# sizhe-li/neural-jacobian-field

Hardware: AMD Instinct MI355X
Metric: rendered rays/s (64 samples/ray, 256^2 image) (higher is better)
Workload: dtype f32 (v_mfma_f32_32x32x2_f32: exact fp32 products, fp32 accumulate -- the reference's arithmetic)

## Files before the change

### neural-jacobian-field_amd/csrc/njf_device.h

```cpp
#pragma once
#include <hip/hip_runtime.h>
#include <stdint.h>

__device__ __forceinline__ float relu_bits(float x) { return __int_as_float(max(__float_as_int(x), 0)); }

typedef float f32x16 __attribute__((ext_vector_type(16)));
typedef float f32x4 __attribute__((ext_vector_type(4)));
typedef _Float16 f16x8 __attribute__((ext_vector_type(8)));
typedef _Float16 f16x16 __attribute__((ext_vector_type(16)));
typedef _Float16 f16x32 __attribute__((ext_vector_type(32)));
typedef int i32x8 __attribute__((ext_vector_type(8)));
typedef int i32x4 __attribute__((ext_vector_type(4)));
typedef int i32x2 __attribute__((ext_vector_type(2)));
typedef unsigned u32x6 __attribute__((ext_vector_type(6)));

#define PREC_F32 0
#define PREC_F16X2 1
#define PREC_F16F6 2
#define PREC_F16 3

#define NJF_WAVES 4
#define NJF_THREADS (NJF_WAVES * 64)
#define NJF_CHUNK 8192

// ... 674 lines not shown
#pragma unroll
      for (int e = 0; e < 4; ++e) {
        if (t == 0) {
          h[m][4 * q + e] = fmaf(v[b % DEPTH][q][e], w[0], h[m][4 * q + e]);
        } else {
          float acc = h[m][4 * q + e];
          asm("v_fmac_f32 %0, %1, %2" : "+v"(acc) : "v"(v[b % DEPTH][q][e]), "v"(w[t]));
          h[m][4 * q + e] = acc;
        }
      }
    asm volatile("" : "+v"(h[m]) : : "memory");
    if (b + DEPTH < NB) issue(b + DEPTH);
    __builtin_amdgcn_sched_barrier(0);
  }
}

#define NJF_F16_GATHER_DEPTH 8
template <int MB, int DEPTH = NJF_F16_GATHER_DEPTH>
__device__ __forceinline__ void add_hoisted_latent_f16(const _Float16* __restrict__ gz, const PointGeom& g, int hh,
                                                       f32x16 (&h)[MB], const Footprint* shared = nullptr) {
  if (!NJF_GATHER) return;
  Footprint f;
  if (shared != nullptr) f = *shared;
  else point_footprint(g, f);
  const _Float16* gb = gz + (size_t)g.gofs + 8 * hh;
  const _Float16* p[4] = {gb + f.t00, gb + f.t01, gb + f.t10, gb + f.t11};
  const float w[4] = {f.w00, f.w01, f.w10, f.w11};
  constexpr int NB = 4 * MB;
  constexpr int D = DEPTH < NB ? DEPTH : NB;
  f16x8 v[D][2];
  auto issue = [&](int b) {
    const _Float16* src = p[b / MB] + 32 * (b % MB);
#pragma unroll
    for (int q = 0; q < 2; ++q) v[b % D][q] = *(const f16x8*)(src + 16 * q);
  };
#pragma unroll
  for (int b = 0; b < D; ++b) issue(b);
#pragma unroll
  for (int b = 0; b < NB; ++b) {
    const int t = b / MB, m = b % MB;
#pragma unroll
    for (int q = 0; q < 2; ++q)
#pragma unroll
      for (int e = 0; e < 8; ++e) h[m][8 * q + e] = fmaf((float)v[b % D][q][e], w[t], h[m][8 * q + e]);
    asm volatile("" : "+v"(h[m]) : : "memory");
    if (b + D < NB) issue(b + D);
    __builtin_amdgcn_sched_barrier(0);
  }
}

struct TileShareF16 {
  unsigned pe[16];
};

__device__ __forceinline__ void share_tile(const f32x16 (&pe)[2], TileShareF16& sh) {
#pragma unroll
  for (int t = 0; t < 4; ++t)
#pragma unroll
    for (int p = 0; p < 4; ++p) sh.pe[4 * t + p] = pack_pair_f16<false>(pe[t >> 1][8 * (t & 1) + 2 * p], pe[t >> 1][8 * (t & 1) + 2 * p + 1]);
}

template <class ST>
__device__ __forceinline__ void mma_lin_in_f16_packed(ST& st, const float* __restrict__ wl, int lane, const unsigned (&pk)[16],
                                                      f32x16 (&out)[4]) {
  const f16x8* base = (const f16x8*)wl + lane;
  constexpr int T = 4;
  f16x8 a[4];
#pragma unroll
  for (int i = 0; i < 4; ++i) a[i] = base[i * 64];
#pragma unroll
  for (int t = 0; t < T; ++t) {
    f16x8 n[4] = {a[0], a[1], a[2], a[3]};
    if (t + 1 < T) {
#pragma unroll
      for (int i = 0; i < 4; ++i) n[i] = base[((t + 1) * 4 + i) * 64];
    }
    dma_issue(st, 2 * t);
    dma_issue(st, 2 * t + 1);
    __builtin_amdgcn_sched_barrier(0);
    const f16x8 b = __builtin_bit_cast(f16x8, u32x4{pk[4 * t], pk[4 * t + 1], pk[4 * t + 2], pk[4 * t + 3]});
#pragma unroll
    for (int m = 0; m < 4; ++m) out[m] = __builtin_amdgcn_mfma_f32_32x32x16_f16(a[m], b, out[m], 0, 0, 0);
#pragma unroll
    for (int i = 0; i < 4; ++i) a[i] = n[i];
  }
}


template <int MB, int PREC, int DEPTH = 4>
__device__ __forceinline__ void add_hoisted_latent(const float* __restrict__ gz, const PointGeom& g, int lane,
                                                   f32x16 (&h)[MB]) {
  if constexpr (PREC == PREC_F16) add_hoisted_latent_f16<MB>((const _Float16*)gz, g, lane >> 5, h);
  else if constexpr (PREC == PREC_F16F6) add_hoisted_latent_quad<MB, DEPTH>(gz, g, lane, h);
  else add_hoisted_latent_half<MB, DEPTH>(gz, g, lane >> 5, h);
}

template <int PREC>
__device__ __forceinline__ const float* map_at(const float* base, size_t elements) {
  if constexpr (PREC == PREC_F16) return (const float*)((const _Float16*)base + elements);
  else return base + elements;
}

__device__ __forceinline__ float sin_accurate(float arg) {
  const float C_HI = 0.15915493667125702f, C_LO = 6.4206382432985265e-09f;
  const float u = arg * C_HI;
  float e = fmaf(arg, C_HI, -u);
  e = fmaf(arg, C_LO, e);
  const float y = (u - rintf(u)) + e;
  return __builtin_amdgcn_sinf(y);
}

__device__ __forceinline__ void positional_encoding(float xc, float yc, float zc, int hh, f32x16 (&pe)[2]) {
#ifdef NJF_ABLATE_PE
  pe[0] = (f32x16)(xc);
  pe[1] = (f32x16)(yc + zc);
  return;
#endif
  const float two_pi = 6.2831855f;
  const float half_pi = hh ? 1.5707964f : 0.0f;
  const float sx[3] = {two_pi * xc, two_pi * yc, two_pi * zc};
#pragma unroll
  for (int s = 0; s < 30; ++s) {
    const int d = s / 10, f = s % 10;
    const float arg = sx[d] * (float)(1 << f) + half_pi;
    pe[s >> 4][s & 15] = sin_accurate(arg);
  }
  pe[1][14] = hh ? zc : xc;
  pe[1][15] = hh ? 1.0f : yc;
}

__device__ __forceinline__ void sh4(float dx, float dy, float dz, float (&o)[16]) {
  const float x = ((dx + 1.0f) / 2.0f) * 2.0f - 1.0f;
  const float y = ((dy + 1.0f) / 2.0f) * 2.0f - 1.0f;
  const float z = ((dz + 1.0f) / 2.0f) * 2.0f - 1.0f;
  const float xy = x * y, xz = x * z, yz = y * z, x2 = x * x, y2 = y * y, z2 = z * z;
  o[0] = 0.28209479177387814f;
  o[1] = -0.48860251190291987f * y;
  o[2] = 0.48860251190291987f * z;
  o[3] = -0.48860251190291987f * x;
  o[4] = 1.0925484305920792f * xy;
  o[5] = -1.0925484305920792f * yz;
  o[6] = 0.94617469575755997f * z2 - 0.31539156525251999f;
  o[7] = -1.0925484305920792f * xz;
  o[8] = 0.54627421529603959f * x2 - 0.54627421529603959f * y2;
  o[9] = 0.59004358992664352f * y * (-3.0f * x2 + y2);
  o[10] = 2.8906114426405538f * xy * z;
  o[11] = 0.45704579946446572f * y * (1.0f - 5.0f * z2);
  o[12] = 0.3731763325901154f * z * (5.0f * z2 - 3.0f);
  o[13] = 0.45704579946446572f * x * (1.0f - 5.0f * z2);
  o[14] = 1.4453057213202769f * z * (x2 - y2);
  o[15] = 0.59004358992664352f * x * (-x2 + 3.0f * y2);
}

template <int KB0, bool RELU, int KBI, class ST>
__device__ __forceinline__ void mma_chunk_gather_f32(ST& st, const float* __restrict__ wl, int lane, const f32x16 (&in)[KBI],
                                                     f32x16 (&out)[4], const float* __restrict__ gz, const PointGeom& g) {
  static_assert(NJF_DMA_ROUNDS == 8, "one DMA round behind every second group of blocks 0 and 1");
  constexpr int DEPTH = 2;
  constexpr int FIRST = 4;
  Footprint f;
  point_footprint(g, f);
  const float* gb = gz + (size_t)g.gofs + 4 * (lane >> 5);
  const float* p[4] = {gb + f.t00, gb + f.t01, gb + f.t10, gb + f.t11};
  const float w[4] = {f.w00, f.w01, f.w10, f.w11};
  f32x4 v[DEPTH][4];
  auto issue = [&](int b) {
    const float* src = p[b & 3] + 32 * (b >> 2);
#pragma unroll
    for (int q = 0; q < 4; ++q) v[b % DEPTH][q] = *(const f32x4*)(src + 8 * q);
  };
  auto fold = [&](int m, int i) {
    const int t = i >> 4, r = i & 15, b = 4 * m + t;
    if (t == 0) {
      out[m][r] = fmaf(v[b % DEPTH][r >> 2][r & 3], w[0], out[m][r]);
    } else {
      float acc = out[m][r];
      asm("v_fmac_f32 %0, %1, %2" : "+v"(acc) : "v"(v[b % DEPTH][r >> 2][r & 3]), "v"(w[t]));
      out[m][r] = acc;
    }
  };
  auto refill = [&](int m, int t) {
    asm volatile("" : "+v"(out[m]) : : "memory");
    if (4 * m + t + DEPTH < 16) issue(4 * m + t + DEPTH);
  };
  auto folded = [](int n) { return n <= FIRST ? 0 : (n - FIRST) * 64 / (32 - FIRST); };
  if (NJF_GATHER) {
#pragma unroll
    for (int b = 0; b < DEPTH; ++b) issue(b);
  }
  const float* base = wl + lane * 4;
  f32x16 bin[2];
  f32x4 a = *(const f32x4*)base;
#pragma unroll
  for (int m = 0; m < 4; ++m) {
#pragma unroll
    for (int kq = 0; kq < 8; ++kq) {
      const int kb = kq >> 2, q = kq & 3, gi = 8 * m + kq;
      f32x4 n = a;
      if (gi + 1 < 32) n = *(const f32x4*)(base + (((gi + 1) & 7) * 4 + ((gi + 1) >> 3)) * 256);
      if (gi < 16 && (gi & 1) == 0) dma_issue(st, gi >> 1);
#pragma unroll
      for (int e = 0; e < 4; ++e) {
        if (m == 0) {
          float b = in[KB0 + kb][q * 4 + e];
          if (RELU) b = relu_bits(b);
          bin[kb][q * 4 + e] = b;
        }
        out[m] = __builtin_amdgcn_mfma_f32_32x32x2f32(a[e], bin[kb][q * 4 + e], out[m], 0, 0, 0);
        if (NJF_GATHER && m > 0) {
#pragma unroll
          for (int i = folded(4 * kq + e); i < folded(4 * kq + e + 1); ++i) fold(m - 1, i);
        }
      }
      if (NJF_GATHER && m > 0) {
#pragma unroll
        for (int t = folded(4 * kq) / 16; t < folded(4 * kq + 4) / 16; ++t) refill(m - 1, t);
      }
      a = n;
      __builtin_amdgcn_sched_barrier(0);
    }
  }
  st.dma_next = NJF_DMA_ROUNDS;
  NJF_STAMP(st, 4);
  if (NJF_GATHER) {
#pragma unroll
    for (int t = 0; t < 4; ++t) {
#pragma unroll
      for (int i = 16 * t; i < 16 * t + 16; ++i) fold(3, i);
      refill(3, t);
      __builtin_amdgcn_sched_barrier(0);
    }
  }
  NJF_STAMP(st, 5);
}

struct ActDump {
  float* act;
  float* pe;
  size_t stride;
  unsigned* mask = nullptr;
  bool half = false;
  float* feat = nullptr;
};

__device__ __forceinline__ float* dump_layer(const ActDump& d, int l) {
  if (d.act == nullptr) return nullptr;
  return d.half ? (float*)((_Float16*)d.act + (size_t)l * d.stride) : d.act + (size_t)l * d.stride;
}

template <bool DO_RELU>
__device__ __forceinline__ void dump_vec128(float* __restrict__ dst, const f32x16 (&v)[4], unsigned* __restrict__ mask = nullptr,
                                            bool half = false) {
  if (dst == nullptr) return;
  if (half) {
    _Float16* d16 = (_Float16*)dst;
#pragma unroll
    for (int m = 0; m < 4; ++m)
#pragma unroll
      for (int q = 0; q < 2; ++q) {
        u32x4 o;
#pragma unroll
        for (int e = 0; e < 4; ++e) o[e] = pack_pair_f16<DO_RELU>(v[m][8 * q + 2 * e], v[m][8 * q + 2 * e + 1]);
        *(u32x4*)(d16 + 16 * m + 8 * q) = o;
      }
  } else {
#pragma unroll
  for (int m = 0; m < 4; ++m)
#pragma unroll
    for (int q = 0; q < 4; ++q) {
      f32x4 o;
#pragma unroll
      for (int e = 0; e < 4; ++e) o[e] = DO_RELU ? fmaxf(v[m][4 * q + e], 0.f) : v[m][4 * q + e];
      *(f32x4*)(dst + 16 * m + 4 * q) = o;
    }
  }
  if (mask != nullptr) {
    unsigned w[2] = {0u, 0u};
#pragma unroll
    for (int m = 0; m < 4; ++m)
#pragma unroll
      for (int r = 0; r < 16; ++r) {
        const unsigned b = (unsigned)min(max(__float_as_int(v[m][r]), 0), 1);
        w[m >> 1] |= b << (16 * (m & 1) + r);
      }
    typedef unsigned u32x2 __attribute__((ext_vector_type(2)));
    *(u32x2*)mask = u32x2{w[0], w[1]};
  }
}

template <int PREC, bool DUMP = false, int SHARED = 0, class ST>
__device__ __forceinline__ void resnet_tile(ST& st, const float* __restrict__ bias,
                                            const float* __restrict__ gz, const PointGeom& g,
                                            const f32x16 (&pe)[2], int wave, int lane, f32x16 (&out)[1],
                                            ActDump dump = ActDump{nullptr, nullptr, 0}, const TileShareF16* share = nullptr) {
  static_assert(SHARED == 0 || (PREC == PREC_F16 && !DUMP), "the shared tile state exists for the plain-fp16 inference kernels");
  const int hh = lane >> 5;
  constexpr bool FUSED = PREC == PREC_F32 && !DUMP;
  f32x16 h[4], net[4];
#pragma unroll
  for (int m = 0; m < 4; ++m) h[m] = (f32x16)(0.f);
  if (DUMP && dump.pe != nullptr) {
#pragma unroll
    for (int kb = 0; kb < 2; ++kb)
#pragma unroll
      for (int q = 0; q < 4; ++q) {
        f32x4 o;
#pragma unroll
        for (int e = 0; e < 4; ++e) o[e] = pe[kb][4 * q + e];
        *(f32x4*)(dump.pe + 16 * kb + 4 * q) = o;
      }
  }
  {
    const float* wl = stream_step(st, wave, lane);
    if constexpr ((SHARED & 1) != 0) mma_lin_in_f16_packed(st, wl, lane, share->pe, h);
    else if constexpr (FUSED) mma_chunk_gather_f32<0, false, 2>(st, wl, lane, pe, h, gz, g);
    else mma_chunk<PREC, 4, 2, 0, false, 2>(st, wl, lane, pe, h);
  }
  if constexpr (PREC == PREC_F16) {
    static_assert(!DUMP, "the plain-fp16 mode is an inference mode (training forwards dump fp32-class activations)");
    Footprint fp_net;
    if constexpr ((SHARED & 2) != 0) point_footprint(g, fp_net);
    for (int blk = 0; blk < 5; ++blk) {
      if (blk < 3) {
        NJF_STAMP(st, 4);
        if constexpr ((SHARED & 2) != 0) add_hoisted_latent_f16<4>((const _Float16*)map_at<PREC>(gz, blk * 128), g, hh, h, &fp_net);
        else add_hoisted_latent<4, PREC>(map_at<PREC>(gz, blk * 128), g, lane, h);
        NJF_STAMP(st, 5);
      }
      const float* bl = bias + blk * 256;
      bias_init<4, true, PREC>(bl, hh, net);
      {
        const float* wl = stream_step(st, wave, lane);
        mma_chunk<PREC, 4, 4, 0, true, 4>(st, wl, lane, h, net);
      }
      if (blk >= 2) bias_init<4, false, PREC, true>(bl + 128, hh, h);
      {
        const float* wl = stream_step(st, wave, lane);
        mma_chunk<PREC, 4, 4, 0, true, 4>(st, wl, lane, net, h);
      }
    }
  } else
  for (int blk = 0; blk < 5; ++blk) {
    if (!FUSED && blk < 3) {
      NJF_STAMP(st, 4);
      add_hoisted_latent<4, PREC>(gz + blk * 128, g, lane, h);
      NJF_STAMP(st, 5);
    }
    if (DUMP) dump_vec128<true>(dump_layer(dump, 2 * blk), h, dump.mask ? dump.mask + (size_t)(2 * blk) * (dump.stride / 32) : nullptr, dump.half);
    const float* bl = bias + blk * 256;
    bias_init<4, true, PREC>(bl, hh, net);
    {
      {
        const float* wl = stream_step(st, wave, lane);
        mma_chunk<PREC, 4, 2, 0, true, 4>(st, wl, lane, h, net);
      }
      {
        const float* wl = stream_step(st, wave, lane);
        mma_chunk<PREC, 4, 2, 2, true, 4>(st, wl, lane, h, net);
      }
    }
    if (DUMP) dump_vec128<true>(dump_layer(dump, 2 * blk + 1), net, dump.mask ? dump.mask + (size_t)(2 * blk + 1) * (dump.stride / 32) : nullptr, dump.half);
    bias_init<4, false, PREC>(bl + 128, hh, h);
    {
      {
        const float* wl = stream_step(st, wave, lane);
        mma_chunk<PREC, 4, 2, 0, true, 4>(st, wl, lane, net, h);
      }
      {
        const float* wl = stream_step(st, wave, lane);
        bool plain = true;
        if constexpr (FUSED) {
          if (blk < 2) {
            mma_chunk_gather_f32<2, true, 4>(st, wl, lane, net, h, gz + (blk + 1) * 128, g);
            plain = false;
          }
        }
        if (plain) mma_chunk<PREC, 4, 2, 2, true, 4>(st, wl, lane, net, h);
      }
    }
    if (DUMP && dump.feat != nullptr) dump_vec128<false>(dump.feat + (size_t)blk * dump.stride, h);
  }
  if (DUMP) dump_vec128<true>(dump_layer(dump, 10), h, dump.mask ? dump.mask + (size_t)10 * (dump.stride / 32) : nullptr, dump.half);
  bias_init<1, true, PREC>(bias + 1280, hh, out);
  {
    const float* wl = stream_step(st, wave, lane);
    mma_chunk<PREC, 1, 4, 0, true, 4>(st, wl, lane, h, out);
  }
}

struct ColorDump {
  float* in;
  float* act;
  size_t stride;
};

template <bool DO_RELU>
__device__ __forceinline__ void dump_vec32(float* __restrict__ dst, const f32x16 (&v)[2]) {
#pragma unroll
  for (int m = 0; m < 2; ++m)
#pragma unroll
    for (int q = 0; q < 4; ++q) {
      f32x4 o;
#pragma unroll
      for (int e = 0; e < 4; ++e) o[e] = DO_RELU ? fmaxf(v[m][4 * q + e], 0.f) : v[m][4 * q + e];
      *(f32x4*)(dst + 16 * m + 4 * q) = o;
    }
}

template <int PREC, bool DUMP = false, class ST>
__device__ __forceinline__ void color_tile(ST& st, const float* __restrict__ bias, const f32x16 (&cin)[1],
                                           int wave, int lane, f32x16 (&rgb)[1],
                                           ColorDump dump = ColorDump{nullptr, nullptr, 0}) {
  const int hh = lane >> 5;
  const float* wl = stream_step(st, wave, lane);
  f32x16 a[2], b[2];
  a[0] = (f32x16)(0.f);
  a[1] = (f32x16)(0.f);
  mma_chunk<PREC, 2, 1, 0, false, 1>(st, wl, lane, cin, a);
  bias_init<2, true, PREC>(bias, hh, b);
  mma_chunk<PREC, 2, 2, 0, true, 2>(st, wl + 2048, lane, a, b);
  bias_init<1, true, PREC>(bias + 64, hh, rgb);
  mma_chunk<PREC, 1, 2, 0, true, 2>(st, wl + 6144, lane, b, rgb);
  if (DUMP && dump.in != nullptr) {
#pragma unroll
    for (int q = 0; q < 4; ++q) {
      f32x4 o;
#pragma unroll
      for (int e = 0; e < 4; ++e) o[e] = cin[0][4 * q + e];
      *(f32x4*)(dump.in + 4 * q) = o;
    }
    dump_vec32<true>(dump.act, a);
    dump_vec32<true>(dump.act + dump.stride, b);
  }
}

__device__ __forceinline__ float erf_branchless(float a) {
  const float t = fabsf(a), s = a * a;
  float r = fmaf(-1.72853470e-5f, t, 3.83197126e-4f);
  const float u = fmaf(-3.88396438e-3f, t, 2.42546219e-2f);
  r = fmaf(r, s, u);
  r = fmaf(r, t, -1.06777877e-1f);
  r = fmaf(r, t, -6.34846687e-1f);
  r = fmaf(r, t, -1.28717512e-1f);
  r = fmaf(r, t, -t);
  const float hi = copysignf(1.0f - __builtin_amdgcn_exp2f(r * 1.4426950408889634f), a);
  float q = -5.96761703e-4f;
  q = fmaf(q, s, 4.99119423e-3f);
  q = fmaf(q, s, -2.67681349e-2f);
  q = fmaf(q, s, 1.12819925e-1f);
  q = fmaf(q, s, -3.76125336e-1f);
  q = fmaf(q, s, 1.28379166e-1f);
  const float lo = fmaf(q, a, a);
  return t > 0.927734375f ? hi : lo;
}

__device__ __forceinline__ float erf_as7126(float a) {
  const float t = __builtin_amdgcn_rcpf(fmaf(0.3275911f, fabsf(a), 1.0f));
  float p = 1.061405429f;
  p = fmaf(p, t, -1.453152027f);
  p = fmaf(p, t, 1.421413741f);
  p = fmaf(p, t, -0.284496736f);
  p = fmaf(p, t, 0.254829592f);
  p *= t;
  const float e = __builtin_amdgcn_exp2f((a * a) * -1.4426950408889634f);
  return copysignf(fmaf(-p, e, 1.0f), a);
}

__device__ __forceinline__ void norm64(const f32x16 (&x)[2], f32x16 (&n)[2]) {
  float s = 0.f;
#pragma unroll
  for (int m = 0; m < 2; ++m)
#pragma unroll
    for (int r = 0; r < 16; ++r) s += x[m][r];
  s += __shfl_xor(s, 32, 64);
  const float mean = s / 64.0f;
  float v = 0.f;
#pragma unroll
  for (int m = 0; m < 2; ++m)
#pragma unroll
    for (int r = 0; r < 16; ++r) {
      const float d = x[m][r] - mean;
      v = fmaf(d, d, v);
    }
  v += __shfl_xor(v, 32, 64);
  const float rstd = __builtin_amdgcn_rsqf(v / 64.0f + 1e-5f);
  const float shift = -mean * rstd;
#pragma unroll
  for (int m = 0; m < 2; ++m)
#pragma unroll
    for (int r = 0; r < 16; ++r) n[m][r] = fmaf(x[m][r], rstd, shift);
}

__device__ __forceinline__ void store_vec64(float* __restrict__ dst, const f32x16 (&v)[2]) {
  if (dst == nullptr) return;
#pragma unroll
  for (int m = 0; m < 2; ++m)
#pragma unroll
    for (int q = 0; q < 4; ++q) {
      f32x4 o;
#pragma unroll
      for (int e = 0; e < 4; ++e) o[e] = v[m][4 * q + e];
      *(f32x4*)(dst + 16 * m + 4 * q) = o;
    }
}
__device__ __forceinline__ void load_vec64(const float* __restrict__ src, bool ok, f32x16 (&v)[2]) {
#pragma unroll
  for (int m = 0; m < 2; ++m)
#pragma unroll
    for (int q = 0; q < 4; ++q) {
      f32x4 o = {0.f, 0.f, 0.f, 0.f};
      if (ok) o = *(const f32x4*)(src + 16 * m + 4 * q);
#pragma unroll
      for (int e = 0; e < 4; ++e) v[m][4 * q + e] = o[e];
    }
}

template <int PREC, class ST>
__device__ __forceinline__ void transformer_tile(ST& st, const float* __restrict__ bias,
                                                 const float* __restrict__ gq, const PointGeom& g,
                                                 const f32x16 (&pe)[2], int keys, int wave, int lane, f32x16 (&out)[1],
                                                 float* __restrict__ xdump = nullptr, size_t xstride = 0) {
  const int hh = lane >> 5;
  f32x16 x[2], n[2], t[2];
  x[0] = (f32x16)(0.f);
  x[1] = (f32x16)(0.f);
  const float* wl = stream_step(st, wave, lane);
  mma_chunk<PREC, 2, 2, 0, false, 2>(st, wl, lane, pe, x);
  add_hoisted_latent<2, PREC>(gq, g, lane, x);
  for (int l = 0; l < 3; ++l) {
    const float* bl = bias + 256 * l;
    if (xdump != nullptr) store_vec64(xdump + (size_t)l * xstride, x);
    norm64(x, n);
    bias_init<2, true, PREC>(bl, hh, t);
// ... 120 lines not shown
```

### neural-jacobian-field_amd/csrc/njf_kernels.hip

```cpp
#include <hip/hip_runtime.h>
#include <math.h>
#include <stdint.h>

#include <atomic>
#include <type_traits>

#include "../../include/njf_hip.h"
#include "njf_device.h"

enum {
  NJF_OK = 0,
  NJF_E_NULL = -1,
  NJF_E_SHAPE = -2,
  NJF_E_ACTION_DIM = -3,
  NJF_E_SAMPLES = -4,
  NJF_E_DOUT = -5,
  NJF_E_MODE = -6,
  NJF_E_GMAP = -7,
  NJF_E_VALUE = -8,
};

extern "C" int njf_abi_version(void) { return NJF_ABI_VERSION; }
extern "C" int njf_rays_per_workgroup(void) { return NJF_WAVES; }

// ... 1075 lines not shown
    if (lane >= o) incl += t;
  }
  float acc = incl - run;
  float* cdf = sc + 256;
  __syncthreads();
  for (int i = 0; i < per; ++i) {
    const int s = i0 + i;
    if (s < s_in) {
      acc += (sc[s] + padper) / wsum;
      cdf[s + 1] = fminf(1.0f, acc);
    }
  }
  if (lane == 0) cdf[0] = 0.f;
  __syncthreads();
  for (int k = lane; k <= s_out; k += 64) {
    const float uk = u[k];
    int lo = 0, hi = s_in + 1;
    while (lo < hi) {
      const int mid = (lo + hi) >> 1;
      if (cdf[mid] <= uk) lo = mid + 1;
      else hi = mid;
    }
    const int below = min(max(lo - 1, 0), s_in), above = min(max(lo, 0), s_in);
    const float c0 = cdf[below], c1 = cdf[above];
    const float g0 = bins_in[below], g1 = bins_in[above];
    float t = (uk - c0) / (c1 - c0);
    if (t != t) t = 0.f;
    t = fminf(fmaxf(t, 0.f), 1.f);
    if (store) bins_out[k] = g0 + t * (g1 - g0);
  }
}

struct ProposalArgs {
  RayCommon rc;
  int gmap_offset;
  const float* w_pack;
  const float* b_pack;
  const float* bins_in;
  int bins_per_ray;
  int s_in;
  const float* u;
  int u_per_ray;
  int s_out;
  float anneal;
  float* bins_out;
  float* weights_out;
  float* density_out;
  NjfActivationDump dump;
};

__device__ __forceinline__ ActDump point_dump(const NjfActivationDump& d, size_t pidx, size_t points, int hh,
                                              const PointGeom& g, int tex0, int texel_stride) {
  float* act = nullptr;
  if (d.act) act = d.act_f16 ? (float*)((_Float16*)d.act + pidx * 128 + 64 * hh) : d.act + pidx * 128 + 64 * hh;
  ActDump dump{act, d.pe + pidx * 64 + 32 * hh, points * 128, d.mask ? d.mask + pidx * 4 + 2 * hh : nullptr, d.act_f16 != 0};
  if (hh == 0 && d.foot_idx != nullptr) {
    Footprint f;
    point_footprint(g, f);
    int* fi = d.foot_idx + pidx * 4;
    fi[0] = tex0 + f.t00 / texel_stride;
    fi[1] = tex0 + f.t01 / texel_stride;
    fi[2] = tex0 + f.t10 / texel_stride;
    fi[3] = tex0 + f.t11 / texel_stride;
    float* fw = d.foot_w + pidx * 4;
    fw[0] = f.w00;
    fw[1] = f.w01;
    fw[2] = f.w10;
    fw[3] = f.w11;
  }
  return dump;
}

template <int PREC, bool DUMP = false>
__global__ void __launch_bounds__(NJF_THREADS, 2) proposal_kernel(ProposalArgs a) {
  const int tid = threadIdx.x;
  const int wave = __builtin_amdgcn_readfirstlane(tid >> 6);
  const int lane = tid & 63, j = lane & 31, hh = lane >> 5;
  const int wg = xcd_remap(blockIdx.x, gridDim.x);
  const int ray = wg * NJF_WAVES + wave;
  const bool ray_ok = ray < a.rc.total_rays;
  const int rayc = min(ray, a.rc.total_rays - 1);
  const int b = rayc / a.rc.rays_per_batch;

  load_bias_block(a.b_pack, NJF_RESNET_B_FLOATS, 0);
  const int tiles = (a.s_in + 31) >> 5;
  WeightStream st;
  stream_begin(st, a.w_pack, resnet_chunks<PREC>(), tiles, wave, lane);
  NJF_STAMP_ARM(st, true, wave);

  CamCtx cam;
  load_ctx(a.rc.cams.ctxt_w2c, a.rc.cams.ctxt_k, b, cam);
  const float near = a.rc.cams.z_near[b], far = a.rc.cams.z_far[b];
  const float ox = a.rc.origins[3 * (size_t)rayc], oy = a.rc.origins[3 * (size_t)rayc + 1],
              oz = a.rc.origins[3 * (size_t)rayc + 2];
  const float dx = a.rc.directions[3 * (size_t)rayc], dy = a.rc.directions[3 * (size_t)rayc + 1],
              dz = a.rc.directions[3 * (size_t)rayc + 2];
  const float* gz = map_at<PREC>(a.rc.gmap.data, (size_t)b * a.rc.gmap.height * a.rc.gmap.width * a.rc.gmap.stride + a.gmap_offset);
  const float* bins = a.bins_in + (a.bins_per_ray ? (size_t)rayc * (a.s_in + 1) : 0);
  float* sc = njf_lds + LDS_SCRATCH_PROPOSAL + wave * LDS_SCRATCH_PER_WAVE;
  const float* bias = njf_lds + LDS_BIAS;

  float carry = 0.f;
  for (int t = 0; t < tiles; ++t) {
    const int s = t * 32 + j;
    const bool valid = s < a.s_in;
    const int sc_i = min(s, a.s_in - 1);
    const float b0 = bins[sc_i], b1 = bins[sc_i + 1];
    const float start = b0 * far + (1.0f - b0) * near;
    const float end = b1 * far + (1.0f - b1) * near;
    const float se = start + end;
    const float px = ox + (dx * se) / 2.0f, py = oy + (dy * se) / 2.0f, pz = oz + (dz * se) / 2.0f;
    PointGeom g;
    point_geometry(cam, px, py, pz, a.rc.gmap.height, a.rc.gmap.width, a.rc.gmap.stride, 0u, g);
    NJF_STAMP_P(st, 10);
    f32x16 pe[2];
    positional_encoding(g.xc, g.yc, g.zc, hh, pe);
    f32x16 out[1];
    ActDump dump{nullptr, nullptr, 0};
    if (DUMP && valid && ray_ok)
      dump = point_dump(a.dump, (size_t)ray * a.s_in + s, (size_t)a.rc.total_rays * a.s_in, hh, g,
                        b * a.rc.gmap.height * a.rc.gmap.width, a.rc.gmap.stride);
    resnet_tile<PREC, DUMP>(st, bias, gz, g, pe, wave, lane, out, dump);
    NJF_STAMP_P(st, 14);
    const float pre = __shfl(out[0][0], j, 64);
    const float sigma = expf(pre - 1.0f);
    const float w = tile_weights(end - start, sigma, valid, j, carry);
    if (valid && hh == 0) {
      float wa = w;
      if (a.anneal != 1.0f) wa = powf(w, a.anneal);
      sc[s] = wa + 0.01f;
      if (ray_ok) {
        if (a.weights_out) a.weights_out[(size_t)ray * a.s_in + s] = w;
        if (a.density_out) a.density_out[(size_t)ray * a.s_in + s] = sigma;
      }
    }
  }
  NJF_STAMP_P(st, 13);
  __syncthreads();
  const float* u = a.u + (a.u_per_ray ? (size_t)rayc * (a.s_out + 1) : 0);
  pdf_resample_ray(sc, bins, a.s_in, u, a.s_out, a.bins_out + (size_t)rayc * (a.s_out + 1), lane, ray_ok);
  NJF_STAMP_FLUSH(st, 15, lane);
}

template <int PREC, int DUMP, int SHARE = 0, class ST>
__device__ __forceinline__ float density_stage(ST& st, const float* __restrict__ gz_d, const PointGeom& g, int wave,
                                               int lane, f32x16 (&geo)[1], ActDump dump, TileShareF16* share = nullptr) {
  const int j = lane & 31, hh = lane >> 5;
  f32x16 pe[2];
  positional_encoding(g.xc, g.yc, g.zc, hh, pe);
  if constexpr (SHARE != 0) {
    share_tile(pe, *share);
    resnet_tile<PREC, false, SHARE>(st, njf_lds + LDS_BIAS, gz_d, g, pe, wave, lane, geo, dump, share);
  } else {
    resnet_tile<PREC, DUMP == 2>(st, njf_lds + LDS_BIAS, gz_d, g, pe, wave, lane, geo, dump);
  }
  return expf(__shfl(geo[0][15], j, 64) - 1.0f);
}

template <int PREC, int DUMP, class ST>
__device__ __forceinline__ void color_stage(ST& st, const f32x16 (&geo)[1], float dirx, float diry, float dirz,
                                            int wave, int lane, float (&rgb)[3], ColorDump cdump) {
  const int j = lane & 31, hh = lane >> 5;
  asm volatile("" : "+v"(dirx), "+v"(diry), "+v"(dirz));
  float sh[16];
  sh4(dirx, diry, dirz, sh);
  f32x16 cin[1], crgb[1];
#pragma unroll
  for (int r = 0; r < 16; ++r) cin[0][r] = hh ? sh[r] : (r < 15 ? geo[0][r] : 1.0f);
  color_tile<PREC, DUMP == 2>(st, njf_lds + LDS_BIAS + NJF_RESNET_B_FLOATS, cin, wave, lane, crgb, cdump);
#pragma unroll
  for (int c = 0; c < 3; ++c) {
    const float x = __shfl(crgb[0][c], j, 64);
    rgb[c] = 1.0f / (1.0f + expf(-x));
  }
}

template <int JKIND, int PREC, int DUMP, int SHARE = 0, class ST>
__device__ __forceinline__ void jacobian_stage(ST& st, const float* __restrict__ gz_j, const PointGeom& g,
                                               const float* __restrict__ action, int action_dim, int wave, int lane,
                                               f32x16 (&jac)[1], float (&flow)[3], ActDump dump, const TileShareF16* share = nullptr) {
  const int hh = lane >> 5;
  const float* bias = njf_lds + LDS_BIAS + NJF_RESNET_B_FLOATS + NJF_COLOR_B_FLOATS;
  if constexpr (SHARE != 0) {
    static_assert(JKIND == 1 && DUMP == 0, "shared tile state: ResnetFC Jacobian head, inference");
    NJF_STAMP(st, 6);
    NJF_STAMP(st, 7);
    f32x16 unused[2];
    resnet_tile<PREC, false, SHARE>(st, bias, gz_j, g, unused, wave, lane, jac, dump, share);
  } else {
  float xc = g.xc, yc = g.yc, zc = g.zc;
  asm volatile("" : "+v"(xc), "+v"(yc), "+v"(zc) : : "memory");
  f32x16 pe[2];
  NJF_STAMP(st, 6);
  positional_encoding(xc, yc, zc, hh, pe);
  NJF_STAMP_PIN("+v"(pe[0]), "+v"(pe[1]));
  NJF_STAMP(st, 7);
  if (JKIND == 1)
    resnet_tile<PREC, DUMP == 1>(st, bias, gz_j, g, pe, wave, lane, jac, dump);
  else {
    if (DUMP == 1 && dump.pe != nullptr) {
#pragma unroll
      for (int kb = 0; kb < 2; ++kb)
#pragma unroll
        for (int q = 0; q < 4; ++q) {
          f32x4 o;
#pragma unroll
          for (int e = 0; e < 4; ++e) o[e] = pe[kb][4 * q + e];
          *(f32x4*)(dump.pe + 16 * kb + 4 * q) = o;
        }
    }
    transformer_tile<PREC>(st, bias, gz_j, g, pe, action_dim, wave, lane, jac, DUMP == 1 ? dump.act : nullptr, dump.stride);
  }
  }
  float ph[3] = {0.f, 0.f, 0.f};
  if (action) {
#pragma unroll
    for (int r = 0; r < 16; ++r) {
      const int d0 = r, d1 = 16 + r;
      const float a0 = (d0 / 3) < action_dim ? action[d0 / 3] : 0.f;
      const float a1 = (d1 / 3) < action_dim ? action[d1 / 3] : 0.f;
      ph[r % 3] = fmaf(jac[0][r], hh ? a1 : a0, ph[r % 3]);
    }
  }
  float mine[3];
#pragma unroll
  for (int s = 0; s < 3; ++s) mine[s] = hh ? ph[(s + 2) % 3] : ph[s];
#pragma unroll
  for (int s = 0; s < 3; ++s) flow[s] = mine[s] + __shfl_xor(mine[s], 32, 64);
}

struct RenderArgs {
  RayCommon rc;
  int goff_d, goff_j;
  const float* w_all;
  const float* b_d;
  const float* b_c;
  const float* b_j;
  const float* bins;
  int samples;
  NjfRenderOutputs out;
};

struct SamplePlace {
  float delta, tm, px, py, pz;
};
__device__ __forceinline__ void place_sample(float b0, float b1, float near, float far, float ox,
                                             float oy, float oz, float dx, float dy, float dz, SamplePlace& sp) {
  asm volatile("" : "+v"(b0), "+v"(b1));
  const float start = b0 * far + (1.0f - b0) * near;
  const float end = b1 * far + (1.0f - b1) * near;
  const float se = start + end;
  sp.delta = end - start;
  sp.tm = se / 2.0f;
  sp.px = ox + (dx * se) / 2.0f;
  sp.py = oy + (dy * se) / 2.0f;
  sp.pz = oz + (dz * se) / 2.0f;
}

template <int JKIND, int PREC, int DUMP = 0, bool AF = true, int PRECJ = PREC>
__global__ void __launch_bounds__(NJF_THREADS, 2) render_kernel(RenderArgs a) {
  constexpr bool WITH_J = JKIND != 0;
  constexpr int J_CHUNKS = JKIND == 1 ? resnet_chunks<PRECJ>() : (JKIND == 2 ? NJF_TRANSFORMER_CHUNKS : 0);
  constexpr int J_BIAS = JKIND == 1 ? NJF_RESNET_B_FLOATS : NJF_TRANSFORMER_B_FLOATS;
  const int tid = threadIdx.x;
  const int wave = __builtin_amdgcn_readfirstlane(tid >> 6);
  const int lane = tid & 63, j = lane & 31, hh = lane >> 5;
  const int wg = xcd_remap(blockIdx.x, gridDim.x);
  const int ray = wg * NJF_WAVES + wave;
  const bool ray_ok = ray < a.rc.total_rays;
  const int rayc = min(ray, a.rc.total_rays - 1);
  const int b = rayc / a.rc.rays_per_batch;
  const int S = a.samples;

  load_bias_block(a.b_d, NJF_RESNET_B_FLOATS, 0);
  load_bias_block(a.b_c, NJF_COLOR_B_FLOATS, NJF_RESNET_B_FLOATS);
  if (WITH_J) load_bias_block(a.b_j, J_BIAS, NJF_RESNET_B_FLOATS + NJF_COLOR_B_FLOATS);
  const int tiles = (S + 31) >> 5;
  WeightStreamT<resnet_gap_at<PREC>(), resnet_gap<PREC>()> st;
  stream_begin(st, a.w_all, resnet_chunks<PREC>() + 1 + J_CHUNKS, tiles, wave, lane);
  NJF_STAMP_ARM(st, false, wave);

  CamCtx cam;
  load_ctx(a.rc.cams.ctxt_w2c, a.rc.cams.ctxt_k, b, cam);
  const float near = a.rc.cams.z_near[b], far = a.rc.cams.z_far[b];
  const float ox = a.rc.origins[3 * (size_t)rayc], oy = a.rc.origins[3 * (size_t)rayc + 1],
              oz = a.rc.origins[3 * (size_t)rayc + 2];
  const float dx = a.rc.directions[3 * (size_t)rayc], dy = a.rc.directions[3 * (size_t)rayc + 1],
              dz = a.rc.directions[3 * (size_t)rayc + 2];
  const size_t gbase = (size_t)b * a.rc.gmap.height * a.rc.gmap.width * a.rc.gmap.stride;
  const float* gz_d = map_at<PREC>(a.rc.gmap.data, gbase + a.goff_d);
  const float* gz_j = map_at<PRECJ>(a.rc.gmap.data, gbase + a.goff_j);
  const float* bins = a.bins + (size_t)rayc * (S + 1);
  const int A = a.rc.cams.action_dim;
  const float* action = a.rc.cams.action ? a.rc.cams.action + (size_t)b * A : nullptr;

  float carry = 0.f;
  float acc_rgb[3] = {0.f, 0.f, 0.f}, acc_w = 0.f, acc_wt = 0.f;
  float acc_p[3] = {0.f, 0.f, 0.f}, acc_pw[3] = {0.f, 0.f, 0.f};
  float tmin = 3.0e38f, tmax = -3.0e38f;
  f32x16 acc_j = (f32x16)(0.f);
  const bool want_af = AF && WITH_J && a.out.action_features != nullptr;

  for (int t = 0; t < tiles; ++t) {
    const int s = t * 32 + j;
    const bool valid = s < S;
    const int sc_i = min(s, S - 1);
    const size_t si = (size_t)ray * S + s;
    const bool store = valid && ray_ok;
    const float bin0 = bins[sc_i], bin1 = bins[sc_i + 1];
    PointGeom g;
    {
      SamplePlace sp;
      place_sample(bin0, bin1, near, far, ox, oy, oz, dx, dy, dz, sp);
      point_geometry(cam, sp.px, sp.py, sp.pz, a.rc.gmap.height, a.rc.gmap.width, a.rc.gmap.stride, 0u, g);
    }
    NJF_STAMP(st, 10);
    ActDump dump{nullptr, nullptr, 0};
    ColorDump cdump{nullptr, nullptr, 0};
    if (DUMP != 0 && store) {
      const size_t points = (size_t)a.rc.total_rays * S;
      const NjfActivationDump d{DUMP == 1 ? a.out.jac_act : a.out.den_act, a.out.jac_pe, a.out.foot_idx, a.out.foot_w,
                                DUMP == 1 ? a.out.jac_mask : a.out.den_mask, a.out.dump_f16};
      dump = point_dump(d, si, points, hh, g, b * a.rc.gmap.height * a.rc.gmap.width, a.rc.gmap.stride);
      if constexpr (JKIND == 2 && DUMP == 1) {
        dump.act = a.out.jac_act ? a.out.jac_act + si * 64 + 32 * hh : nullptr;
        dump.stride = points * 64;
        dump.mask = nullptr;
        dump.half = false;
      }
      if (DUMP == 2) cdump = ColorDump{a.out.col_in + si * 32 + 16 * hh, a.out.col_act + si * 64 + 32 * hh, points * 64};
    }
    f32x16 geo[1];
#define NJF_F16_SHARE_D 1
#define NJF_F16_SHARE_J 3
    constexpr int SHARE_D = (PREC == PREC_F16 && DUMP == 0 && !AF) ? NJF_F16_SHARE_D : 0;
    constexpr int SHARE_J = (SHARE_D != 0 && JKIND == 1 && PRECJ == PREC_F16) ? NJF_F16_SHARE_J : 0;
    TileShareF16 share;
    const float sigma = density_stage<PREC, DUMP, SHARE_D>(st, gz_d, g, wave, lane, geo, DUMP == 2 ? dump : ActDump{nullptr, nullptr, 0}, &share);
    float w;
    {
      SamplePlace sp;
      place_sample(bin0, bin1, near, far, ox, oy, oz, dx, dy, dz, sp);
      NJF_STAMP(st, 14);
      w = tile_weights(sp.delta, sigma, valid, j, carry);
      NJF_STAMP_PIN("+v"(w));
      NJF_STAMP(st, 15);
      if (valid) {
        acc_w += w;
        acc_wt = fmaf(w, sp.tm, acc_wt);
        tmin = fminf(tmin, sp.tm);
        tmax = fmaxf(tmax, sp.tm);
// ... 3812 lines not shown
```

Measured before the change: 2.034 million.

## Carry gather tail and bias init into next chunk's MFMA stream in fp32 resnet

Generalizes the fp32 gather-fused MMA chunk into a side-work template. The tail of the latent-grid gather fold, which previously ran after the MFMA loop, is carried as state into the next block's first chunk so it overlaps with that block's MFMAs. Bias initialization for the following output blocks is also interleaved into the MFMA loop. This should hide VALU and load latency behind the matrix pipe, at the cost of more live registers and more complex scheduling. The new path is only used for non-dump (inference) fp32 forwards.

```diff
diff --git a/neural-jacobian-field_amd/csrc/njf_device.h b/neural-jacobian-field_amd/csrc/njf_device.h
--- a/neural-jacobian-field_amd/csrc/njf_device.h
+++ b/neural-jacobian-field_amd/csrc/njf_device.h
@@ -850,44 +850,84 @@
   o[15] = 0.59004358992664352f * x * (-x2 + 3.0f * y2);
 }
 
-template <int KB0, bool RELU, int KBI, class ST>
-__device__ __forceinline__ void mma_chunk_gather_f32(ST& st, const float* __restrict__ wl, int lane, const f32x16 (&in)[KBI],
-                                                     f32x16 (&out)[4], const float* __restrict__ gz, const PointGeom& g) {
+enum { SIDE_NONE = 0, SIDE_GATHER = 1, SIDE_CARRY = 2, SIDE_BIAS = 3, SIDE_GATHER_TAIL = 4 };
+
+struct GatherCarry {
+  f32x4 v[2][4];
+  const float* p[2];
+  float w[4];
+};
+struct ChunkSide {
+  GatherCarry* gc = nullptr;
+  const float* gz = nullptr;
+  const PointGeom* g = nullptr;
+  f32x16* tail = nullptr;
+  const float* bias = nullptr;
+};
+
+template <bool ASSIGN>
+__device__ __forceinline__ void bias_block(const float* __restrict__ bl, int hh, int m, f32x16& acc) {
+  f32x16 one[1] = {acc};
+  bias_init<1, ASSIGN, PREC_F32>(bl + 48 * hh + 16 * m, hh, one);
+  acc = one[0];
+}
+
+template <int SIDE, int KB0, bool RELU, int KBI, class ST>
+__device__ __forceinline__ void mma_chunk_f32(ST& st, const float* __restrict__ wl, int lane, const f32x16 (&in)[KBI],
+                                              f32x16 (&out)[4], const ChunkSide side = ChunkSide{}) {
   static_assert(NJF_DMA_ROUNDS == 8, "one DMA round behind every second group of blocks 0 and 1");
+  static_assert(SIDE != SIDE_CARRY || KB0 == 0, "the carried fold writes h[3]: the chunk must not read it");
+  constexpr bool ANY_GATHER = SIDE == SIDE_GATHER || SIDE == SIDE_GATHER_TAIL;
+  constexpr bool GATHER = NJF_GATHER && ANY_GATHER, CARRY = NJF_GATHER && SIDE == SIDE_CARRY;
   constexpr int DEPTH = 2;
   constexpr int FIRST = 4;
-  Footprint f;
-  point_footprint(g, f);
-  const float* gb = gz + (size_t)g.gofs + 4 * (lane >> 5);
-  const float* p[4] = {gb + f.t00, gb + f.t01, gb + f.t10, gb + f.t11};
-  const float w[4] = {f.w00, f.w01, f.w10, f.w11};
+  const float* p[4];
+  float w[4];
   f32x4 v[DEPTH][4];
+  if constexpr (GATHER) {
+    Footprint f;
+    point_footprint(*side.g, f);
+    const float* gb = side.gz + (size_t)side.g->gofs + 4 * (lane >> 5);
+    p[0] = gb + f.t00, p[1] = gb + f.t01, p[2] = gb + f.t10, p[3] = gb + f.t11;
+    w[0] = f.w00, w[1] = f.w01, w[2] = f.w10, w[3] = f.w11;
+  }
+  if constexpr (CARRY) {
+    p[2] = side.gc->p[0], p[3] = side.gc->p[1];
+#pragma unroll
+    for (int t = 0; t < 4; ++t) w[t] = side.gc->w[t];
+#pragma unroll
+    for (int s = 0; s < DEPTH; ++s)
+#pragma unroll
+      for (int q = 0; q < 4; ++q) v[s][q] = side.gc->v[s][q];
+  }
   auto issue = [&](int b) {
     const float* src = p[b & 3] + 32 * (b >> 2);
 #pragma unroll
     for (int q = 0; q < 4; ++q) v[b % DEPTH][q] = *(const f32x4*)(src + 8 * q);
   };
-  auto fold = [&](int m, int i) {
-    const int t = i >> 4, r = i & 15, b = 4 * m + t;
+  auto fold = [&](f32x16& o, int i) {
+    const int t = i >> 4, r = i & 15;
     if (t == 0) {
-      out[m][r] = fmaf(v[b % DEPTH][r >> 2][r & 3], w[0], out[m][r]);
+      o[r] = fmaf(v[t % DEPTH][r >> 2][r & 3], w[0], o[r]);
     } else {
-      float acc = out[m][r];
-      asm("v_fmac_f32 %0, %1, %2" : "+v"(acc) : "v"(v[b % DEPTH][r >> 2][r & 3]), "v"(w[t]));
-      out[m][r] = acc;
+      float acc = o[r];
+      asm("v_fmac_f32 %0, %1, %2" : "+v"(acc) : "v"(v[t % DEPTH][r >> 2][r & 3]), "v"(w[t]));
+      o[r] = acc;
     }
   };
-  auto refill = [&](int m, int t) {
-    asm volatile("" : "+v"(out[m]) : : "memory");
+  auto refill = [&](f32x16& o, int m, int t) {
+    asm volatile("" : "+v"(o) : : "memory");
     if (4 * m + t + DEPTH < 16) issue(4 * m + t + DEPTH);
   };
   auto folded = [](int n) { return n <= FIRST ? 0 : (n - FIRST) * 64 / (32 - FIRST); };
-  if (NJF_GATHER) {
+  auto carried = [](int n) { return n <= FIRST ? 0 : (n <= 20 ? 2 * (n - FIRST) : (n <= 32 ? 32 : (n <= 64 ? n : 64))); };
+  if constexpr (GATHER) {
 #pragma unroll
     for (int b = 0; b < DEPTH; ++b) issue(b);
   }
   const float* base = wl + lane * 4;
   f32x16 bin[2];
+  f32x16 bnext;
   f32x4 a = *(const f32x4*)base;
 #pragma unroll
   for (int m = 0; m < 4; ++m) {
@@ -897,39 +937,79 @@
       f32x4 n = a;
       if (gi + 1 < 32) n = *(const f32x4*)(base + (((gi + 1) & 7) * 4 + ((gi + 1) >> 3)) * 256);
       if (gi < 16 && (gi & 1) == 0) dma_issue(st, gi >> 1);
+      if constexpr (SIDE == SIDE_BIAS) {
+        if (kq == 0 && m > 0) {
+#pragma unroll
+          for (int r = 0; r < 16; ++r) out[m][r] += bnext[r];
+        }
+      }
 #pragma unroll
       for (int e = 0; e < 4; ++e) {
-        if (m == 0) {
-          float b = in[KB0 + kb][q * 4 + e];
+        float b;
+        if constexpr (ANY_GATHER) {
+          if (m == 0) {
+            b = in[KB0 + kb][q * 4 + e];
+            if (RELU) b = relu_bits(b);
+            bin[kb][q * 4 + e] = b;
+          }
+          b = bin[kb][q * 4 + e];
+        } else {
+          b = in[KB0 + kb][q * 4 + e];
           if (RELU) b = relu_bits(b);
-          bin[kb][q * 4 + e] = b;
-        }
-        out[m] = __builtin_amdgcn_mfma_f32_32x32x2f32(a[e], bin[kb][q * 4 + e], out[m], 0, 0, 0);
-        if (NJF_GATHER && m > 0) {
-#pragma unroll
-          for (int i = folded(4 * kq + e); i < folded(4 * kq + e + 1); ++i) fold(m - 1, i);
-        }
-      }
-      if (NJF_GATHER && m > 0) {
-#pragma unroll
-        for (int t = folded(4 * kq) / 16; t < folded(4 * kq + 4) / 16; ++t) refill(m - 1, t);
+        }
+        out[m] = __builtin_amdgcn_mfma_f32_32x32x2f32(a[e], b, out[m], 0, 0, 0);
+        if constexpr (GATHER) {
+          if (m > 0) {
+#pragma unroll
+            for (int i = folded(4 * kq + e); i < folded(4 * kq + e + 1); ++i) fold(out[m - 1], i);
+          }
+        }
+        if constexpr (CARRY) {
+#pragma unroll
+          for (int i = carried(4 * gi + e); i < carried(4 * gi + e + 1); ++i) fold(*side.tail, i);
+        }
+      }
+      if constexpr (GATHER) {
+        if (m > 0) {
+#pragma unroll
+          for (int t = folded(4 * kq) / 16; t < folded(4 * kq + 4) / 16; ++t) refill(out[m - 1], m - 1, t);
+        }
+      }
+      if constexpr (CARRY) {
+#pragma unroll
+        for (int t = carried(4 * gi) / 16; t < carried(4 * gi + 4) / 16; ++t) refill(*side.tail, 3, t);
+      }
+      if constexpr (SIDE == SIDE_CARRY) {
+        if (kq == 7 && (m == 1 || m == 2)) bias_block<true>(side.bias, lane >> 5, m + 1, out[m + 1]);
+      }
+      if constexpr (SIDE == SIDE_BIAS) {
+        if (kq == 7 && m < 3) bias_block<true>(side.bias, lane >> 5, m + 1, bnext);
       }
       a = n;
       __builtin_amdgcn_sched_barrier(0);
     }
   }
   st.dma_next = NJF_DMA_ROUNDS;
-  NJF_STAMP(st, 4);
-  if (NJF_GATHER) {
+  if constexpr (GATHER && SIDE == SIDE_GATHER_TAIL) {
+    NJF_STAMP(st, 4);
 #pragma unroll
     for (int t = 0; t < 4; ++t) {
 #pragma unroll
-      for (int i = 16 * t; i < 16 * t + 16; ++i) fold(3, i);
-      refill(3, t);
+      for (int i = 16 * t; i < 16 * t + 16; ++i) fold(out[3], i);
+      refill(out[3], 3, t);
       __builtin_amdgcn_sched_barrier(0);
     }
-  }
-  NJF_STAMP(st, 5);
+    NJF_STAMP(st, 5);
+  }
+  if constexpr (GATHER && SIDE == SIDE_GATHER) {
+#pragma unroll
+    for (int t = 0; t < 4; ++t) side.gc->w[t] = w[t];
+    side.gc->p[0] = p[2], side.gc->p[1] = p[3];
+#pragma unroll
+    for (int s = 0; s < DEPTH; ++s)
+#pragma unroll
+      for (int q = 0; q < 4; ++q) side.gc->v[s][q] = v[s][q];
+  }
 }
 
 struct ActDump {
@@ -986,7 +1066,7 @@
   }
 }
 
-template <int PREC, bool DUMP = false, int SHARED = 0, class ST>
+template <int PREC, bool DUMP = false, int SHARED = 0, bool SCHED = true, class ST>
 __device__ __forceinline__ void resnet_tile(ST& st, const float* __restrict__ bias,
                                             const float* __restrict__ gz, const PointGeom& g,
                                             const f32x16 (&pe)[2], int wave, int lane, f32x16 (&out)[1],
@@ -994,6 +1074,8 @@
   static_assert(SHARED == 0 || (PREC == PREC_F16 && !DUMP), "the shared tile state exists for the plain-fp16 inference kernels");
   const int hh = lane >> 5;
   constexpr bool FUSED = PREC == PREC_F32 && !DUMP;
+  constexpr int LATENTS = 3;
+  GatherCarry gc;
   f32x16 h[4], net[4];
 #pragma unroll
   for (int m = 0; m < 4; ++m) h[m] = (f32x16)(0.f);
@@ -1011,7 +1093,7 @@
   {
     const float* wl = stream_step(st, wave, lane);
     if constexpr ((SHARED & 1) != 0) mma_lin_in_f16_packed(st, wl, lane, share->pe, h);
-    else if constexpr (FUSED) mma_chunk_gather_f32<0, false, 2>(st, wl, lane, pe, h, gz, g);
+    else if constexpr (FUSED) mma_chunk_f32<SCHED ? SIDE_GATHER : SIDE_GATHER_TAIL, 0, false, 2>(st, wl, lane, pe, h, ChunkSide{&gc, gz, &g});
     else mma_chunk<PREC, 4, 2, 0, false, 2>(st, wl, lane, pe, h);
   }
   if constexpr (PREC == PREC_F16) {
@@ -1037,6 +1119,49 @@
         mma_chunk<PREC, 4, 4, 0, true, 4>(st, wl, lane, net, h);
       }
     }
+  } else {
+  if constexpr (FUSED && SCHED) {
+    auto block = [&](int blk, auto carry_in, auto gather_out) __attribute__((always_inline)) {
+      constexpr bool CARRY_IN = decltype(carry_in)::value, GATHER_OUT = decltype(gather_out)::value;
+      const float* bl = bias + blk * 256;
+      if constexpr (CARRY_IN) {
+        bias_block<true>(bl, hh, 0, net[0]);
+        bias_block<true>(bl, hh, 1, net[1]);
+      } else {
+        bias_init<4, true, PREC>(bl, hh, net);
+      }
+      {
+        const float* wl = stream_step(st, wave, lane);
+        if constexpr (CARRY_IN) {
+          ChunkSide side;
+          side.gc = &gc, side.tail = &h[3], side.bias = bl;
+          mma_chunk_f32<SIDE_CARRY, 0, true, 4>(st, wl, lane, h, net, side);
+        } else {
+          mma_chunk_f32<SIDE_NONE, 0, true, 4>(st, wl, lane, h, net);
+        }
+      }
+      {
+        const float* wl = stream_step(st, wave, lane);
+        mma_chunk_f32<SIDE_NONE, 2, true, 4>(st, wl, lane, h, net);
+      }
+      bias_block<false>(bl + 128, hh, 0, h[0]);
+      {
+        const float* wl = stream_step(st, wave, lane);
+        ChunkSide side;
+        side.bias = bl + 128;
+        mma_chunk_f32<SIDE_BIAS, 0, true, 4>(st, wl, lane, net, h, side);
+      }
+      {
+        const float* wl = stream_step(st, wave, lane);
+        if constexpr (GATHER_OUT) mma_chunk_f32<SIDE_GATHER, 2, true, 4>(st, wl, lane, net, h, ChunkSide{&gc, gz + (blk + 1) * 128, &g});
+        else mma_chunk_f32<SIDE_NONE, 2, true, 4>(st, wl, lane, net, h);
+      }
+    };
+#pragma nounroll
+    for (int blk = 0; blk + 1 < LATENTS; ++blk) block(blk, std::true_type{}, std::true_type{});
+    block(LATENTS - 1, std::true_type{}, std::false_type{});
+#pragma nounroll
+    for (int blk = LATENTS; blk < 5; ++blk) block(blk, std::false_type{}, std::false_type{});
   } else
   for (int blk = 0; blk < 5; ++blk) {
     if (!FUSED && blk < 3) {
@@ -1069,7 +1194,7 @@
         bool plain = true;
         if constexpr (FUSED) {
           if (blk < 2) {
-            mma_chunk_gather_f32<2, true, 4>(st, wl, lane, net, h, gz + (blk + 1) * 128, g);
+            mma_chunk_f32<SIDE_GATHER_TAIL, 2, true, 4>(st, wl, lane, net, h, ChunkSide{&gc, gz + (blk + 1) * 128, &g});
             plain = false;
           }
         }
@@ -1077,6 +1202,7 @@
       }
     }
     if (DUMP && dump.feat != nullptr) dump_vec128<false>(dump.feat + (size_t)blk * dump.stride, h);
+  }
   }
   if (DUMP) dump_vec128<true>(dump_layer(dump, 10), h, dump.mask ? dump.mask + (size_t)10 * (dump.stride / 32) : nullptr, dump.half);
   bias_init<1, true, PREC>(bias + 1280, hh, out);
diff --git a/neural-jacobian-field_amd/csrc/njf_kernels.hip b/neural-jacobian-field_amd/csrc/njf_kernels.hip
--- a/neural-jacobian-field_amd/csrc/njf_kernels.hip
+++ b/neural-jacobian-field_amd/csrc/njf_kernels.hip
@@ -1251,7 +1251,7 @@
     share_tile(pe, *share);
     resnet_tile<PREC, false, SHARE>(st, njf_lds + LDS_BIAS, gz_d, g, pe, wave, lane, geo, dump, share);
   } else {
-    resnet_tile<PREC, DUMP == 2>(st, njf_lds + LDS_BIAS, gz_d, g, pe, wave, lane, geo, dump);
+    resnet_tile<PREC, DUMP == 2, 0, DUMP == 0>(st, njf_lds + LDS_BIAS, gz_d, g, pe, wave, lane, geo, dump);
   }
   return expf(__shfl(geo[0][15], j, 64) - 1.0f);
 }
@@ -1295,7 +1295,7 @@
   NJF_STAMP_PIN("+v"(pe[0]), "+v"(pe[1]));
   NJF_STAMP(st, 7);
   if (JKIND == 1)
-    resnet_tile<PREC, DUMP == 1>(st, bias, gz_j, g, pe, wave, lane, jac, dump);
+    resnet_tile<PREC, DUMP == 1, 0, DUMP == 0>(st, bias, gz_j, g, pe, wave, lane, jac, dump);
   else {
     if (DUMP == 1 && dump.pe != nullptr) {
 #pragma unroll
```

Result: no change. 2.054 million, median of 6 (+1.0%).
